# david-wb/tiny-diffusion

Hardware: AMD Instinct MI355X
Metric: train images/s (q_sample+fwd+MSE+bwd+allreduce+Adam), MNIST 28x28 UNet fp32; 1000-step sample latency in `sample` (higher is better)
Workload: dtype f32; 1 GPU; diffusion.py unconditional MNIST 28x28 UNet, fp32, train step, batch 256/GPU (BASELINE.json configs[1]); global_batch=256, per_gpu_batch=256, parallelism=dp1

## Files before the change

### tiny_diffusion_amd/csrc/unet.hip

```cpp
#include "internal.h"
#include <algorithm>
#include <cstdlib>
#include <mutex>
#include <new>
#include <string>
#include <vector>

namespace {

struct UnitDef {
  int cin, cout, hw;
  int in_bn;
  int cin_real;
};

struct NetSpec {
  int in_ch, hw0, out_hw;
  int x0_ch, x0_real;
  int overlap;
  int time_dim;
  int enc_hw[4];
  int dec_hw[3];
  int skip_ch[3];
  UnitDef units[13];
// ... 72 lines not shown
    bnscr = std::max(bnscr, tdx_bn_relu_bwd_scratch_floats((int64_t)b * d.hw * d.hw, d.cout));
    gbuf = std::max(gbuf, b * d.hw * d.hw * (size_t)std::max(d.cin, d.cout));
  }
  for (int k = 0; k < 3; ++k) {
    const int hp = S.enc_hw[k + 1];
    L.ep[k] = take(b * hp * hp * S.skip_ch[k]);
  }
  for (int k = 0; k < 3; ++k) {
    const UnitDef& d = S.units[7 + 2 * k];
    L.cat[k] = take(b * d.hw * d.hw * d.cin);
  }
  L.d1a = take(b * S.out_hw * S.out_hw * 64);
  gbuf = std::max(gbuf, b * (size_t)S.out_hw * S.out_hw * 64);
  L.stats = take(stats);
  L.ksplit_floats = ksplit;
  L.ksplit = take(ksplit);
  L.gbuf = gbuf;
  L.G1 = take(gbuf); L.G2 = take(gbuf); L.G3 = take(gbuf); L.G4 = take(gbuf);
  for (int k = 0; k < 3; ++k) {
    L.GS[k] = take(b * S.enc_hw[k] * S.enc_hw[k] * S.skip_ch[k]);
    L.gtp[k] = take(b * S.skip_ch[k]);
  }
  L.slabs = take(slabs);
  L.slabs2 = take(slabs);
  L.bnscr = take(bnscr);
  L.smallp = take((size_t)tdx_small_conv_wgrad_blocks(B, S.hw0, S.hw0) * tdx_small_conv_partial_width());
  L.smallp2 = take((size_t)tdx_small_conv_wgrad_blocks(B, S.hw0, S.hw0) * tdx_small_conv_partial_width());
  L.timescr = take(3 * b * S.time_dim);
  L.total = o;
  return L;
}

}

struct PlanHandles {
  hipStream_t side, side2, half;
  hipEvent_t ev[81];
};

struct tdx_unet {
  int max_batch, num_classes, kind;
  NetSpec spec_own;
  const NetSpec* spec;
  float* wpack;
  size_t wf_off[13], wd_off[13];
  float* upack;
  size_t uf_off[13], ud_off[13];
  bool wino_f[13], wino_d[13], wino_w[13];
  float* infer_ss;
  size_t iss_off[13];
  bool packed;
  bool wf_tiled;
  float* tab;
  size_t tab_floats;
  int tab_T, tab_batch, tab_gen, pack_gen;
  const void* tab_cond;
  const int64_t* tab_tau;
  bool skip_time_path;
  PStep ps;
  bool whole_batch;
  hipStream_t half_own;
  hipEvent_t ev_h_fork, ev_h_join;
  PlanHandles handles;
  int precision, saved_precision;
  int io16, saved_io16;
  tdx_allreduce_fn bn_sync;
  void* bn_sync_user;
  double* bn_sync_buf;
  int saved_batch, saved_mode;
  float* g_next;
  int bw_unit, bw_nblk;
  float* g_x;
  struct GBuf { float* p; int w_unit; int s2; int age; } gb[4];
  int clock;
  bool red_pending[13];
  bool materialize;
  int use_streams;
  hipStream_t side_own, side2_own;
  hipStream_t side;
  hipEvent_t ev_dy[13], ev_w[13], ev_join, ev_fork, ev_pack;
  hipStream_t side2;
  hipEvent_t ev_s2_fork[3], ev_s2_done[3], ev_join2, ev_red[13];
  hipEvent_t ev_mark[N_STAGES][2];
};

static std::mutex g_handles_mu;
static std::vector<PlanHandles> g_handles_pool;

static bool make_handles(PlanHandles* h) {
  {
    std::lock_guard<std::mutex> lk(g_handles_mu);
    if (!g_handles_pool.empty()) { *h = g_handles_pool.back(); g_handles_pool.pop_back(); return true; }
  }
  int lo = 0, hi = 0;
  (void)hipDeviceGetStreamPriorityRange(&lo, &hi);
  h->side = h->side2 = h->half = nullptr;
  if (hipStreamCreateWithPriority(&h->side, hipStreamNonBlocking, lo) != hipSuccess) return false;
  if (hipStreamCreateWithPriority(&h->side2, hipStreamNonBlocking, lo) != hipSuccess) return false;
  if (hipStreamCreateWithFlags(&h->half, hipStreamNonBlocking) != hipSuccess) return false;
  for (auto& e : h->ev)
    if (hipEventCreateWithFlags(&e, hipEventDisableTiming) != hipSuccess) return false;
  return true;
}

static void recycle_handles(const PlanHandles& h) {
  (void)hipStreamSynchronize(h.side);
  (void)hipStreamSynchronize(h.side2);
  (void)hipStreamSynchronize(h.half);
  std::lock_guard<std::mutex> lk(g_handles_mu);
  g_handles_pool.push_back(h);
}

extern "C" int tdx_unet_create_ex(tdx_unet** out, int max_batch, int kind, int num_classes) {
  return tdx_unet_create_hw(out, max_batch, kind, num_classes, 0);
}

extern "C" int tdx_unet_create_hw(tdx_unet** out, int max_batch, int kind, int num_classes, int hw) {
  return tdx_unet_create_full(out, max_batch, kind, num_classes, hw, 0);
}

extern "C" int tdx_unet_create_full(tdx_unet** out, int max_batch, int kind, int num_classes, int hw,
                                    int time_dim) {
  if (!out || max_batch <= 0 || num_classes < 0 || kind < 0 || kind > 2 || hw < 0 || time_dim < 0) return TDX_E_BADARG;
  if (kind == TDX_UNET_LATENT_MLP && time_dim != 0 && time_dim != 256) return TDX_E_SHAPE;
  if (kind == TDX_UNET_LAION && num_classes != 0) return TDX_E_BADARG;
  if (kind == TDX_UNET_LATENT_MLP && num_classes <= 0) return TDX_E_BADARG;
  NetSpec spec_hw;
  if (kind != TDX_UNET_LATENT_MLP) {
    if (!make_spec(kind, hw, time_dim, &spec_hw)) return TDX_E_SHAPE;
    const NetSpec& S = spec_hw;
    for (int i = 0; i < 13; ++i)
      if (!tdx_conv3x3_shape_ok(max_batch, S.units[i].hw, S.units[i].hw, S.units[i].cin, S.units[i].cout))
        return TDX_E_SHAPE;
  }
  tdx_unet* u = new (std::nothrow) tdx_unet();
  if (!u) return TDX_E_BADARG;
  u->max_batch = max_batch;
  u->num_classes = num_classes;
  u->kind = kind;
  if (kind != TDX_UNET_LATENT_MLP) u->spec_own = spec_hw;
  u->spec = kind == TDX_UNET_LATENT_MLP ? nullptr : &u->spec_own;
  size_t o = 64, so = 0;
  if (u->spec) {
    for (int i = 0; i < 13; ++i) {
      const UnitDef& d = u->spec->units[i];
      const size_t n = (size_t)d.cin * d.cout * 9;
      u->wf_off[i] = o; o += align64(n);
      u->wd_off[i] = o; o += align64(n);
      u->iss_off[i] = so; so += align64(2 * (size_t)d.cout);
    }
  } else {
    so = tdx_latent_infer_ss_floats();
  }
  hipError_t e = hipMalloc(&u->wpack, o * sizeof(float));
  if (e != hipSuccess) { delete u; return (int)e; }
  u->upack = nullptr;
  for (int i = 0; i < 13; ++i) u->wino_f[i] = u->wino_d[i] = u->wino_w[i] = false;
  if (u->spec) {
    size_t uo = 64;
    for (int i = 0; i < 13; ++i) {
      const size_t n = (size_t)u->spec->units[i].cin * u->spec->units[i].cout * 16;
      u->uf_off[i] = uo; uo += align64(n);
      u->ud_off[i] = uo; uo += align64(n);
    }
    e = hipMalloc(&u->upack, uo * sizeof(float));
    if (e != hipSuccess) { (void)hipFree(u->wpack); delete u; return (int)e; }
  }
  e = hipMalloc(&u->infer_ss, so * sizeof(float));
  if (e != hipSuccess) { (void)hipFree(u->wpack); if (u->upack) (void)hipFree(u->upack); delete u; return (int)e; }
  u->packed = false;
  u->wf_tiled = false;
  u->tab = nullptr;
  u->tab_floats = 0;
  u->tab_T = u->tab_batch = 0;
  u->tab_gen = -1;
  u->pack_gen = 0;
  u->tab_cond = nullptr;
  u->tab_tau = nullptr;
  u->skip_time_path = false;
  u->whole_batch = false;
  u->ps = {};
  u->precision = TDX_PREC_F32;
  u->saved_precision = TDX_PREC_F32;
  u->io16 = u->saved_io16 = 0;
  u->bn_sync = nullptr;
  u->bn_sync_user = nullptr;
  u->bn_sync_buf = nullptr;
  u->saved_batch = 0;
  u->saved_mode = -1;
  u->g_next = nullptr;
  u->g_x = nullptr;
  u->bw_unit = -1;
  u->bw_nblk = 0;
  u->materialize = g_knobs.materialize != 0;
  u->use_streams = g_knobs.streams < 0 ? (u->spec ? u->spec->overlap : 0) : g_knobs.streams;
  if (!make_handles(&u->handles)) {
    (void)hipFree(u->wpack); if (u->upack) (void)hipFree(u->upack); (void)hipFree(u->infer_ss);
    delete u;
    return TDX_E_STATE;
  }
  {
    const PlanHandles& h = u->handles;
    int k = 0;
    u->side_own = h.side; u->side2_own = h.side2; u->half_own = h.half;
    for (int i = 0; i < 13; ++i) { u->ev_dy[i] = h.ev[k++]; u->ev_w[i] = h.ev[k++]; u->ev_red[i] = h.ev[k++]; }
    for (int i = 0; i < 3; ++i) { u->ev_s2_fork[i] = h.ev[k++]; u->ev_s2_done[i] = h.ev[k++]; }
    u->ev_join = h.ev[k++]; u->ev_fork = h.ev[k++]; u->ev_pack = h.ev[k++]; u->ev_join2 = h.ev[k++];
    u->ev_h_fork = h.ev[k++]; u->ev_h_join = h.ev[k++];
    for (int i = 0; i < N_STAGES; ++i) { u->ev_mark[i][0] = h.ev[k++]; u->ev_mark[i][1] = h.ev[k++]; }
  }
  u->side = u->side_own;
  u->side2 = u->side2_own;
  *out = u;
  return 0;
}

extern "C" int tdx_unet_create(tdx_unet** out, int max_batch, int num_classes) {
  return tdx_unet_create_ex(out, max_batch, 0, num_classes);
}

extern "C" int tdx_unet_set_bn_sync(tdx_unet* u, tdx_allreduce_fn fn, void* user, double* buffer) {
  if (!u || (fn && !buffer)) return TDX_E_BADARG;
  if (!u->spec) return fn ? TDX_E_SHAPE : 0;
  u->bn_sync = fn;
  u->bn_sync_user = user;
  u->bn_sync_buf = buffer;
  return 0;
}

extern "C" int tdx_unet_set_streams(tdx_unet* u, int mode) {
  if (!u || mode < -1 || mode > 2) return TDX_E_BADARG;
  u->use_streams = mode < 0 ? (u->spec ? u->spec->overlap : 0) : mode;
  return 0;
}

extern "C" int tdx_unet_set_precision(tdx_unet* u, int precision) {
  if (!u || (precision != TDX_PREC_F32 && precision != TDX_PREC_BF16)) return TDX_E_BADARG;
  if (!u->spec) { u->precision = precision; return 0; }
  if (precision != u->precision) u->packed = false;
  u->precision = precision;
  u->io16 = precision == TDX_PREC_BF16 && g_knobs.bf16_storage ? 1 : 0;
  return 0;
}

extern "C" int tdx_unet_destroy(tdx_unet* u) {
  if (!u) return TDX_E_BADARG;
  recycle_handles(u->handles);
  (void)hipFree(u->wpack);
  if (u->upack) (void)hipFree(u->upack);
  (void)hipFree(u->infer_ss);
  if (u->tab) (void)hipFree(u->tab);
  delete u;
  return 0;
}

extern "C" size_t tdx_unet_workspace_bytes(const tdx_unet* u, int batch, int mode) {
  (void)mode;
  if (!u || batch <= 0 || batch > u->max_batch) return 0;
  if (!u->spec) return tdx_latent_workspace_floats(batch) * sizeof(float);
  const size_t whole = make_layout(*u->spec, batch).total;
  const int b0 = (batch + 1) / 2;
  const size_t halves = batch >= 2 ? make_layout(*u->spec, b0).total + make_layout(*u->spec, batch - b0).total : 0;
  return std::max(whole, halves) * sizeof(float);
}

extern "C" int tdx_unet_backward_stages(void) { return N_STAGES; }

extern "C" int tdx_unet_tensor(const tdx_unet* u, int batch, const char* name, size_t* offset_floats,
                               size_t* numel) {
  if (!u || !name || !offset_floats || !numel || batch <= 0 || batch > u->max_batch) return TDX_E_BADARG;
  if (!u->spec) return tdx_latent_tensor(batch, name, offset_floats, numel);
  const NetSpec& S = *u->spec;
  const Layout L = make_layout(S, batch);
  const size_t b = (size_t)batch;
  std::string n(name);
  auto unit_index = [&](const std::string& s, size_t prefix) -> int {
    if (s.size() <= prefix) return -1;
    int v = atoi(s.c_str() + prefix);
    return (v >= 0 && v < 13) ? v : -1;
  };
  auto sq = [](int v) { return (size_t)v * v; };
  struct { const char* nm; size_t off, cnt; } fixed[] = {
      {"x0", L.x0, b * sq(S.hw0) * S.x0_ch},
      {"e1p", L.ep[0], b * sq(S.enc_hw[1]) * S.skip_ch[0]},
      {"e2p", L.ep[1], b * sq(S.enc_hw[2]) * S.skip_ch[1]},
      {"e3p", L.ep[2], b * sq(S.enc_hw[3]) * S.skip_ch[2]},
      {"cat3", L.cat[0], b * sq(S.units[7].hw) * S.units[7].cin},
      {"cat2", L.cat[1], b * sq(S.units[9].hw) * S.units[9].cin},
      {"cat1", L.cat[2], b * sq(S.units[11].hw) * S.units[11].cin},
      {"d1a", L.d1a, b * sq(S.out_hw) * 64}, {"emb", L.emb, b * S.time_dim},
      {"t_copy", L.t, 2 * b}, {"tf", L.sin, b}, {"pre", L.pre, b * S.time_dim},
      {"time_g_h", L.timescr + 2 * b * S.time_dim, b * S.time_dim},
      {"t1", L.tp[0], b * S.skip_ch[0]}, {"t2", L.tp[1], b * S.skip_ch[1]}, {"t3", L.tp[2], b * S.skip_ch[2]},
      {"G1", L.G1, L.gbuf}, {"G2", L.G2, L.gbuf}, {"G3", L.G3, L.gbuf}, {"G4", L.G4, L.gbuf},
      {"GS1", L.GS[0], b * sq(S.enc_hw[0]) * S.skip_ch[0]},
// ... 43 lines not shown
    u->wino_d[i] = tdx_conv3x3_train_algo(B, d.hw, d.hw, d.cin, d.cout, 1) != 0;
    u->wino_w[i] = tdx_conv3x3_train_algo(B, d.hw, d.hw, d.cin, d.cout, 2) != 0;
  }
}

static int pack_units(tdx_unet* u, const float* const* P, int lo, int hi, tdx_stream_t stream, bool tiled, bool infer) {
  TdxPackBatch pb{};
  TdxWinoPackBatch wb{};
  for (int i = lo; i < hi; ++i) {
    const UnitDef& d = u->spec->units[i];
    const bool need_f = infer || !u->wino_f[i], need_d = !infer && !u->wino_d[i];
    if (need_f || need_d) {
      const int k = pb.count++;
      pb.w[k] = P[TDX_P_UNIT0 + 4 * i];
      pb.wf[k] = need_f ? u->wpack + u->wf_off[i] : nullptr;
      pb.wd[k] = need_d && !tiled ? u->wpack + u->wd_off[i] : nullptr;
      pb.cout[k] = d.cout; pb.cin[k] = d.cin; pb.cin_real[k] = d.cin_real;
    }
    if (u->wino_f[i] || u->wino_d[i]) {
      const int k = wb.count++;
      wb.w[k] = P[TDX_P_UNIT0 + 4 * i];
      wb.uf[k] = u->wino_f[i] ? u->upack + u->uf_off[i] : nullptr;
      wb.ud[k] = u->wino_d[i] ? u->upack + u->ud_off[i] : nullptr;
      wb.cout[k] = d.cout; wb.cin[k] = d.cin; wb.cin_real[k] = d.cin_real;
    }
  }
  if (pb.count) {
    auto pack = u->precision == TDX_PREC_BF16 ? tdx_pack_conv3x3_batch_bf16 : tiled ? tdx_pack_conv3x3_tiled_batch : tdx_pack_conv3x3_batch;
    int rc = pack(&pb, stream);
    if (rc) return rc;
  }
  if (wb.count) return tdx_pack_conv3x3_wino_batch(&wb, stream);
  return 0;
}

static int pack_impl(tdx_unet* u, const void* const* params, void* const* buffers,
                     tdx_stream_t stream, bool overlap = false, int train_batch = 0) {
  const float* const* P = reinterpret_cast<const float* const*>(params);
  if (!u->spec) {
    if (buffers) {
      int rc = tdx_latent_pack(P, buffers, u->infer_ss, to_stream(stream));
      if (rc) return rc;
    }
    u->packed = buffers != nullptr;
    ++u->pack_gen;
    return 0;
  }
  const bool tiled = buffers && !overlap && u->precision != TDX_PREC_BF16 && g_knobs.infer_ring;
  u->wf_tiled = tiled;
  decide_wino(u, train_batch, train_batch > 0);
  {
    int rc = pack_units(u, P, 0, overlap ? 2 : 13, stream, tiled, buffers != nullptr && !overlap);
    if (rc) return rc;
  }
  for (int i = 0; i < 13; ++i) {
    const UnitDef& d = u->spec->units[i];
    int rc = 0;
    if (buffers) {
      float* ss = u->infer_ss + u->iss_off[i];
      rc = tdx_bn_finalize(nullptr, 0, 0, 0, d.cout, P[TDX_P_UNIT0 + 4 * i + 2],
                           P[TDX_P_UNIT0 + 4 * i + 3], (float*)buffers[3 * i],
                           (float*)buffers[3 * i + 1], nullptr, ss, ss + d.cout, nullptr,
                           nullptr, 0, stream);
      if (rc) return rc;
    }
  }
  u->packed = buffers != nullptr;
  ++u->pack_gen;
  return 0;
}

extern "C" int tdx_unet_pack(tdx_unet* u, const void* const* params, void* const* buffers,
                             tdx_stream_t stream) {
  if (!u || !params || !buffers) return TDX_E_BADARG;
  return pack_impl(u, params, buffers, stream);
}

static int pack_tail(tdx_unet* u, const void* const* params, tdx_stream_t stream) {
  const float* const* P = reinterpret_cast<const float* const*>(params);
  TDX_HIP(hipEventRecord(u->ev_fork, to_stream(stream)));
  TDX_HIP(hipStreamWaitEvent(u->side, u->ev_fork, 0));
  int rc = pack_units(u, P, 2, 13, reinterpret_cast<tdx_stream_t>(u->side), false, false);
  if (rc) return rc;
  TDX_HIP(hipEventRecord(u->ev_pack, u->side));
  return 0;
}

#define RC(call)            \
  do {                      \
    int rc__ = (call);      \
    if (rc__) return rc__;  \
  } while (0)

static bool infer_halves(const tdx_unet* u, int batch, size_t workspace_bytes, int* b0) {
  if (!u->spec || !u->half_own || u->whole_batch || !g_knobs.sample_halves || batch < 2 || batch < g_knobs.sample_halves_min) return false;
  const int h0 = (batch + 1) / 2;
  if (workspace_bytes < (make_layout(*u->spec, h0).total + make_layout(*u->spec, batch - h0).total) * sizeof(float)) return false;
  *b0 = h0;
  return true;
}

static int unet_forward_impl(tdx_unet* u, const void* const* params, void* const* buffers, const float* x,
                             const int64_t* t, const void* cond, float* out, void* workspace, size_t workspace_bytes,
                             int batch, int mode, tdx_stream_t stream, const PStep& ps);

extern "C" int tdx_unet_forward(tdx_unet* u, const void* const* params, void* const* buffers,
                                const float* x, const int64_t* t, const void* cond, float* out,
                                void* workspace, size_t workspace_bytes, int batch, int mode,
                                tdx_stream_t stream) {
  if (!u || !params || !buffers || !x || !t || !out || !workspace) return TDX_E_BADARG;
  if (batch <= 0 || batch > u->max_batch) return TDX_E_BADARG;
  if (mode < TDX_MODE_TRAIN || mode > TDX_MODE_INFER) return TDX_E_BADARG;
  const bool needs_cond = u->kind == 1 || u->num_classes > 0;
  if (needs_cond != (cond != nullptr)) return TDX_E_BADARG;
  int b0 = 0;
  if (mode == TDX_MODE_INFER && infer_halves(u, batch, workspace_bytes, &b0)) {
    const NetSpec& S = *u->spec;
    if (!u->packed) RC(pack_impl(u, params, buffers, stream));
    hipStream_t st = to_stream(stream);
    const size_t per = (size_t)S.in_ch * S.hw0 * S.hw0;
    const size_t w0 = make_layout(S, b0).total;
    const void* cond1 = !cond ? nullptr
                        : u->kind == 1 ? static_cast<const void*>(static_cast<const float*>(cond) + (size_t)b0 * S.time_dim)
                                       : static_cast<const void*>(static_cast<const int64_t*>(cond) + b0);
    PStep ps0 = u->ps, ps1 = u->ps;
    if (ps1.x) {
      ps1.x += b0 * per;
      if (ps1.z) ps1.z += b0 * per;
      ps1.elem0 = (int64_t)(b0 * per);
      ps1.counter_dec = nullptr;
    }
    TDX_HIP(hipEventRecord(u->ev_h_fork, st));
    TDX_HIP(hipStreamWaitEvent(u->half_own, u->ev_h_fork, 0));
    RC(unet_forward_impl(u, params, buffers, x, t, cond, out, workspace, w0 * sizeof(float), b0, mode, stream, ps0));
    RC(unet_forward_impl(u, params, buffers, x + b0 * per, t + b0, cond1, out + b0 * per,
                         reinterpret_cast<float*>(workspace) + w0, workspace_bytes - w0 * sizeof(float), batch - b0, mode,
                         reinterpret_cast<tdx_stream_t>(u->half_own), ps1));
    TDX_HIP(hipEventRecord(u->ev_h_join, u->half_own));
    TDX_HIP(hipStreamWaitEvent(st, u->ev_h_join, 0));
    return 0;
  }
  return unet_forward_impl(u, params, buffers, x, t, cond, out, workspace, workspace_bytes, batch, mode, stream, u->ps);
}

static int unet_forward_impl(tdx_unet* u, const void* const* params, void* const* buffers, const float* x,
                             const int64_t* t, const void* cond, float* out, void* workspace, size_t workspace_bytes,
                             int batch, int mode, tdx_stream_t stream, const PStep& ps) {
  if (!u->spec) {
    if (workspace_bytes < tdx_latent_workspace_floats(batch) * sizeof(float)) return TDX_E_WORKSPACE;
    if (mode == TDX_MODE_INFER && !u->packed) {
      int rc = pack_impl(u, params, buffers, stream);
      if (rc) return rc;
    }
    int rc = tdx_latent_forward(reinterpret_cast<const float* const*>(params), buffers, x, t,
                                static_cast<const int64_t*>(cond), out, reinterpret_cast<float*>(workspace), batch,
                                mode, u->infer_ss, to_stream(stream), u->precision == TDX_PREC_BF16);
    if (rc) return rc;
    u->saved_batch = mode == TDX_MODE_INFER ? 0 : batch;
    u->saved_mode = mode;
    u->saved_precision = u->precision;
    return 0;
  }
  const NetSpec& S = *u->spec;
  const Layout L = make_layout(S, batch);
  if (workspace_bytes < L.total * sizeof(float)) return TDX_E_WORKSPACE;
  const float* const* P = reinterpret_cast<const float* const*>(params);
  float* ws = reinterpret_cast<float*>(workspace);
  hipStream_t st = to_stream(stream);
  u->side = u->use_streams == 1 ? u->side_own : st;
  u->side2 = u->use_streams ? u->side2_own : st;
  const int B = batch;
  const bool infer = mode == TDX_MODE_INFER;
  const bool training = mode == TDX_MODE_TRAIN;
  const int64_t* labels = u->kind == 0 ? static_cast<const int64_t*>(cond) : nullptr;
  const float* cond_emb = u->kind == 1 ? static_cast<const float*>(cond) : nullptr;

  const bool bf16 = u->precision == TDX_PREC_BF16;
  const int io16 = bf16 ? u->io16 : 0;
  if (!infer) RC(pack_impl(u, params, nullptr, stream, true, B));
  else if (!u->packed) RC(pack_impl(u, params, buffers, stream));
  if (!infer) {
    const size_t nx = (size_t)B * S.hw0 * S.hw0 * S.in_ch;
    const float* src[3] = {x, reinterpret_cast<const float*>(t), reinterpret_cast<const float*>(labels)};
    float* dst[3] = {ws + L.x, ws + L.t, ws + L.y};
    const size_t cnt[3] = {nx, 2 * (size_t)B, labels ? 2 * (size_t)B : 0};
    RC(tdx_copy_segments(src, dst, cnt, 3, st));
  }

  hipStream_t tst = st;
  if (!infer && u->side2 != st) {
    TDX_HIP(hipEventRecord(u->ev_fork, st));
    TDX_HIP(hipStreamWaitEvent(u->side2, u->ev_fork, 0));
    tst = u->side2;
  }
  if (!(infer && u->skip_time_path))
    RC(tdx_time_embed_fwd(u->kind, t, labels, cond_emb, P, ws + L.sin, ws + L.pre, ws + L.emb, ws + L.tp[0],
                          ws + L.tp[1], ws + L.tp[2], B, tst, S.time_dim));
  RC(tdx_initial_conv_fwd(x, P[TDX_P_INIT_W], P[TDX_P_INIT_B], ws + L.x0, B, S.hw0, S.hw0, S.in_ch,
                          S.x0_real, st, io16));

  auto sc = [&](int i) -> const float* { return infer ? nullptr : ws + L.ss[i]; };
  auto sh = [&](int i) -> const float* { return infer ? nullptr : ws + L.ss[i] + S.units[i].cout; };

  auto finalize_bn = [&](int i, int tiles, int tile_rows, int64_t count) -> int {
    const UnitDef& d = S.units[i];
    float* ss = ws + L.ss[i];
    if (training && u->bn_sync) {
      RC(tdx_bn_moments(ws + L.stats, tiles, tile_rows, count, d.cout, u->bn_sync_buf, st));
      RC(u->bn_sync(u->bn_sync_user, u->bn_sync_buf, 2 * d.cout + 1, stream));
      return tdx_bn_finalize_moments(u->bn_sync_buf, d.cout, P[TDX_P_UNIT0 + 4 * i + 2], P[TDX_P_UNIT0 + 4 * i + 3],
                                     (float*)buffers[3 * i], (float*)buffers[3 * i + 1], (int64_t*)buffers[3 * i + 2],
                                     ss, ss + d.cout, ss + 2 * d.cout, ss + 3 * d.cout, st);
    }
    return tdx_bn_finalize(ws + L.stats, tiles, tile_rows, count, d.cout, P[TDX_P_UNIT0 + 4 * i + 2],
                           P[TDX_P_UNIT0 + 4 * i + 3], (float*)buffers[3 * i], (float*)buffers[3 * i + 1],
                           (int64_t*)buffers[3 * i + 2], ss, ss + d.cout, ss + 2 * d.cout, ss + 3 * d.cout,
                           training ? 1 : 0, stream);
  };

  auto run_unit = [&](int i, const float* in, TdxSplitDefer* defer = nullptr, TdxPoolFuse* pool = nullptr) -> int {
    const UnitDef& d = S.units[i];
    const float* wf = u->wpack + u->wf_off[i];
    const float* bias = P[TDX_P_UNIT0 + 4 * i + 1];
    float* Y = ws + L.Y[i];
    float* ss = ws + L.ss[i];
    if (bf16) {
      const int64_t M = (int64_t)B * d.hw * d.hw;
      const bool mat16 = io16 && u->materialize && g_knobs.bf16_materialize;
      if (infer) {
        const float* iss = u->infer_ss + u->iss_off[i];
        return tdx_conv3x3_fwd_bf16_io(in, wf, bias, Y, B, d.hw, d.hw, d.cin, d.cout, TDX_CONV_OUT_BNRELU, nullptr,
                                       nullptr, iss, iss + d.cout, nullptr, io16, stream);
      }
      const bool on_load = d.in_bn && !mat16;
      if (d.in_bn && mat16) in = ws + L.A[i - 1];
      const int fl = (on_load ? TDX_CONV_IN_BNRELU : 0) | (training ? TDX_CONV_OUT_STATS : 0);
      RC(tdx_conv3x3_fwd_bf16_io(in, wf, bias, Y, B, d.hw, d.hw, d.cin, d.cout, fl, on_load ? sc(i - 1) : nullptr,
                                 on_load ? sh(i - 1) : nullptr, nullptr, nullptr, ws + L.stats, io16, stream));
      const int rows = tdx_conv3x3_bf16_stat_tile_rows();
      RC(finalize_bn(i, cdiv(M, rows), rows, M));
      if (mat16 && i + 1 < 13 && S.units[i + 1].in_bn)
        RC(tdx_bn_relu_apply(Y, ws + L.A[i], M, d.cout, ss, ss + d.cout, st, 1));
      return 0;
    }
    if (infer) {
      const float* iss = u->infer_ss + u->iss_off[i];
      if (u->wino_f[i] && tdx_conv3x3_infer_algo(B, d.hw, d.hw, d.cin, d.cout))
        return tdx_conv3x3_fwd_wino_infer_ex(in, u->upack + u->uf_off[i], bias, Y, B, d.hw, d.hw, d.cin, d.cout, iss,
                                             iss + d.cout, ws + L.G1, 2 * L.gbuf, stream, defer, pool);
      if (u->wf_tiled)
        return tdx_conv3x3_fwd_infer_ex(in, wf, bias, Y, B, d.hw, d.hw, d.cin, d.cout, iss, iss + d.cout, ws + L.G1,
                                        2 * L.gbuf, stream, defer, pool);
      return tdx_conv3x3_fwd_splitk_fused(in, wf, bias, Y, B, d.hw, d.hw, d.cin, d.cout, TDX_CONV_OUT_BNRELU, iss,
                                          iss + d.cout, ws + L.G1, 2 * L.gbuf, stream, defer, pool);
    }
    const bool bn_on_load = d.in_bn && !u->materialize;
    if (d.in_bn && u->materialize) in = ws + L.A[i - 1];
    int flags = (bn_on_load ? TDX_CONV_IN_BNRELU : 0) | (training ? TDX_CONV_OUT_STATS : 0);
    if (u->wino_f[i] && !bn_on_load) {
      RC(tdx_conv3x3_fwd_wino(in, u->upack + u->uf_off[i], bias, Y, B, d.hw, d.hw, d.cin, d.cout,
                              training ? TDX_CONV_OUT_STATS : 0, nullptr, nullptr, ws + L.stats, stream));
      RC(finalize_bn(i, tdx_conv3x3_wino_stat_tiles(B, d.hw, d.hw), tdx_conv3x3_wino_stat_tile_rows(B, d.hw, d.hw),
                     (int64_t)B * d.hw * d.hw));
      if (u->materialize && i + 1 < 13 && S.units[i + 1].in_bn)
        RC(tdx_bn_relu_apply(Y, ws + L.A[i], (int64_t)B * d.hw * d.hw, d.cout, ss, ss + d.cout, st));
      return 0;
    }
    if (bn_on_load)
      RC(tdx_conv3x3_fwd(in, wf, bias, Y, B, d.hw, d.hw, d.cin, d.cout, flags, sc(i - 1), sh(i - 1), nullptr, nullptr,
                         ws + L.stats, stream));
    else
      RC(tdx_conv3x3_fwd_train(in, wf, bias, Y, B, d.hw, d.hw, d.cin, d.cout, flags, ws + L.stats, ws + L.ksplit,
                               L.ksplit_floats, stream));
    const int tiles = tdx_conv3x3_stat_tiles(B, d.hw, d.hw, d.cin, d.cout);
    RC(finalize_bn(i, tiles, tdx_conv3x3_stat_tile_rows(B, d.hw, d.hw, d.cin, d.cout), (int64_t)B * d.hw * d.hw));
    if (u->materialize && i + 1 < 13 && S.units[i + 1].in_bn)
      RC(tdx_bn_relu_apply(Y, ws + L.A[i], (int64_t)B * d.hw * d.hw, d.cout, ss, ss + d.cout, st));
    return 0;
  };

  RC(run_unit(0, ws + L.x0));
  if (!infer) RC(pack_tail(u, params, stream));
  for (int k = 0; k < 3; ++k) {
    const int ua = 2 * k, ub = 2 * k + 1;
    if (k == 1 && !infer) TDX_HIP(hipStreamWaitEvent(st, u->ev_pack, 0));
    if (k > 0) RC(run_unit(ua, ws + L.ep[k - 1]));
    TdxPoolFuse pf{infer && !bf16 && (g_knobs.sample_fuse & 2) ? ws + L.ep[k] : nullptr};
    RC(run_unit(ub, ws + L.Y[ua], nullptr, pf.pooled ? &pf : nullptr));
    if (!infer) {
      const int kd = 2 - k, ud = 7 + 2 * kd;
      const UnitDef& dd = S.units[ud];
      const int c_up = S.units[kd == 0 ? 6 : 6 + 2 * kd].cout;
      TDX_HIP(hipEventRecord(u->ev_s2_fork[k], st));
      TDX_HIP(hipStreamWaitEvent(u->side2, u->ev_s2_fork[k], 0));
      RC(tdx_bilinear_ac_fwd_t(ws + L.Y[ub], sc(ub), sh(ub), ws + L.tp[k], ws + L.cat[kd], B, S.enc_hw[k],
                               S.enc_hw[k], dd.hw, dd.hw, S.skip_ch[k], dd.cin, c_up, io16,
                               reinterpret_cast<tdx_stream_t>(u->side2)));
      TDX_HIP(hipEventRecord(u->ev_s2_done[k], u->side2));
    }
    if (!pf.pooled)
      RC(tdx_maxpool2_ceil_fwd_t(ws + L.Y[ub], sc(ub), sh(ub), ws + L.ep[k], B, S.enc_hw[k], S.enc_hw[k],
                                 S.skip_ch[k], io16, stream));
  }
  const bool defer_ok = infer && !bf16 && (g_knobs.sample_fuse & 1);
  TdxSplitDefer dfr{};
  RC(run_unit(6, ws + L.ep[2], defer_ok ? &dfr : nullptr));
  for (int k = 0; k < 3; ++k) {
    const int ua = 7 + 2 * k, ub = 8 + 2 * k;
    const int prev = k == 0 ? 6 : 6 + 2 * k;
    const int skip_u = 5 - 2 * k;
    const int skip_k = 2 - k;
    const UnitDef& da = S.units[ua];
    const UnitDef& dp = S.units[prev];
    const int hw = da.hw, c_up = dp.cout, c_skip = S.skip_ch[skip_k];
    if (infer) {
      RC(tdx_bilinear_pair_fwd_ex(ws + L.Y[prev], &dfr, dp.hw, dp.hw, c_up, ws + L.Y[skip_u], ws + L.tp[skip_k],
                                  S.enc_hw[skip_k], S.enc_hw[skip_k], c_skip, ws + L.cat[k], B, hw, hw, st, io16));
      dfr = TdxSplitDefer{};
    } else {
      RC(tdx_bilinear_ac_fwd_t(ws + L.Y[prev], sc(prev), sh(prev), nullptr, ws + L.cat[k], B, dp.hw, dp.hw, hw, hw,
                               c_up, da.cin, 0, io16, stream));
      TDX_HIP(hipStreamWaitEvent(st, u->ev_s2_done[skip_k], 0));
    }
    RC(run_unit(ua, ws + L.cat[k]));
    RC(run_unit(ub, ws + L.Y[ua], defer_ok ? &dfr : nullptr));
  }
  if (dfr.splits > 0)
    RC(tdx_bilinear_pair_fwd_ex(nullptr, &dfr, S.dec_hw[2], S.dec_hw[2], 64, nullptr, nullptr, 0, 0, 0, ws + L.d1a, B,
                                S.out_hw, S.out_hw, st));
  else
    RC(tdx_bilinear_ac_fwd_t(ws + L.Y[12], sc(12), sh(12), nullptr, ws + L.d1a, B, S.dec_hw[2], S.dec_hw[2],
                             S.out_hw, S.out_hw, 64, 64, 0, io16, stream));
  if (infer && ps.x)
    RC(tdx_final_conv_fwd_psample(ws + L.d1a, P[TDX_P_FINAL_W], P[TDX_P_FINAL_B], out, B, S.out_hw, S.out_hw, S.in_ch,
                                  ps, st, io16));
  else
    RC(tdx_final_conv_fwd(ws + L.d1a, P[TDX_P_FINAL_W], P[TDX_P_FINAL_B], out, B, S.out_hw, S.out_hw, S.in_ch, st, io16));

  u->saved_batch = infer ? 0 : B;
  if (!infer) u->g_x = nullptr;
  u->saved_mode = mode;
  u->saved_precision = u->precision;
  u->saved_io16 = io16;
  return 0;
}

static int unet_backward_impl(tdx_unet* u, const void* const* params, void* const* grads, const float* d_out,
                              void* workspace, size_t workspace_bytes, int batch, int stage_lo, int stage_hi,
                              tdx_stream_t stream);

extern "C" int tdx_unet_backward(tdx_unet* u, const void* const* params, void* const* grads,
                                 const float* d_out, void* workspace, size_t workspace_bytes,
                                 int batch, int stage_lo, int stage_hi, tdx_stream_t stream) {
  if (!u || !params || !grads || !d_out || !workspace) return TDX_E_BADARG;
  const int rc = unet_backward_impl(u, params, grads, d_out, workspace, workspace_bytes, batch, stage_lo, stage_hi, stream);
  if (rc) u->g_x = nullptr;
  return rc;
}

static int unet_backward_impl(tdx_unet* u, const void* const* params, void* const* grads, const float* d_out,
                              void* workspace, size_t workspace_bytes, int batch, int stage_lo, int stage_hi,
                              tdx_stream_t stream) {
  if (batch != u->saved_batch || u->saved_mode == TDX_MODE_INFER || u->saved_mode < 0) return TDX_E_STATE;
  if (stage_lo < 0 || stage_hi > N_STAGES || stage_lo >= stage_hi) return TDX_E_BADARG;
  if (!u->spec) {
    if (workspace_bytes < tdx_latent_workspace_floats(batch) * sizeof(float)) return TDX_E_WORKSPACE;
    return tdx_latent_backward(reinterpret_cast<const float* const*>(params), reinterpret_cast<float* const*>(grads),
                               d_out, reinterpret_cast<float*>(workspace), batch,
                               u->saved_mode == TDX_MODE_TRAIN ? 1 : 0, stage_lo, stage_hi, u->num_classes,
                               to_stream(stream), u->saved_precision == TDX_PREC_BF16);
  }
  const NetSpec& S = *u->spec;
  const Layout L = make_layout(S, batch);
  if (workspace_bytes < L.total * sizeof(float)) return TDX_E_WORKSPACE;
  const float* const* P = reinterpret_cast<const float* const*>(params);
  float* const* G = reinterpret_cast<float* const*>(grads);
  float* ws = reinterpret_cast<float*>(workspace);
  hipStream_t st = to_stream(stream);
  u->side = u->use_streams == 1 ? u->side_own : st;
  u->side2 = u->use_streams ? u->side2_own : st;
  const int B = batch;
  const int training = u->saved_mode == TDX_MODE_TRAIN ? 1 : 0;
  if (u->precision != u->saved_precision) return TDX_E_STATE;
  const bool bf16 = u->saved_precision == TDX_PREC_BF16;
  const int io16 = u->saved_io16;
  typedef tdx_unet::GBuf GBuf;
  GBuf* gb = u->gb;
  int& clock = u->clock;
  if (stage_lo == 0) {
    float* base[4] = {ws + L.G1, ws + L.G2, ws + L.G3, ws + L.G4};
    for (int i = 0; i < 4; ++i) gb[i] = GBuf{base[i], -1, -1, 0};
    clock = 0;
    for (int i = 0; i < 13; ++i) u->red_pending[i] = false;
    u->bw_unit = -1;
  } else if (gb[0].p != ws + L.G1) {
    return TDX_E_STATE;
  }
  auto find = [&](const float* p) -> GBuf* {
    for (int i = 0; i < 4; ++i)
      if (gb[i].p == p) return &gb[i];
    return nullptr;
  };
  auto touch = [&](const float* p) { if (GBuf* b = find(p)) b->age = ++clock; };
  auto acquire = [&](const float* a, const float* b, float** out) -> int {
    GBuf* best = nullptr;
    for (int i = 0; i < 4; ++i) {
      GBuf& c = gb[i];
      if (c.p != a && c.p != b && (!best || c.age < best->age)) best = &c;
    }
    if (best->w_unit >= 0) TDX_HIP(hipStreamWaitEvent(st, u->ev_w[best->w_unit], 0));
    if (best->s2 >= 0) TDX_HIP(hipStreamWaitEvent(st, u->ev_s2_done[best->s2], 0));
    best->w_unit = -1;
    best->s2 = -1;
    best->age = ++clock;
    *out = best->p;
    return 0;
  };
  if (stage_lo > 0 && !find(u->g_next)) return TDX_E_STATE;
  float* g_next = u->g_next;

  tdx_stream_t side = reinterpret_cast<tdx_stream_t>(u->side);
  hipStreamCaptureStatus cap_status = hipStreamCaptureStatusNone;
  (void)hipStreamIsCapturing(st, &cap_status);
  const bool capturing = cap_status == hipStreamCaptureStatusActive;
  auto unit_bwd = [&](int i, const float* in, float** g_in_out) -> int {
    const UnitDef& d = S.units[i];
    float* g = g_next;
    const float* ss = ws + L.ss[i];
    const int64_t rows = (int64_t)B * d.hw * d.hw;
    if (u->bw_unit == i && u->bw_nblk > 0) {
      RC(tdx_bn_relu_bwd_tail(g, ws + L.Y[i], rows, d.cout, ss, ss + d.cout, ss + 2 * d.cout, ss + 3 * d.cout,
                              P[TDX_P_UNIT0 + 4 * i + 2], G[TDX_P_UNIT0 + 4 * i + 2], G[TDX_P_UNIT0 + 4 * i + 3],
                              G[TDX_P_UNIT0 + 4 * i + 1], ws + L.bnscr, u->bw_nblk,
                              ws + L.bnscr + (size_t)u->bw_nblk * 2 * d.cout, training,
                              training ? u->bn_sync : nullptr, u->bn_sync_user, u->bn_sync_buf, stream, io16));
    } else {
      RC(tdx_bn_relu_bwd_sync(g, ws + L.Y[i], rows, d.cout, ss, ss + d.cout, ss + 2 * d.cout,
                              ss + 3 * d.cout, P[TDX_P_UNIT0 + 4 * i + 2], G[TDX_P_UNIT0 + 4 * i + 2],
                              G[TDX_P_UNIT0 + 4 * i + 3], G[TDX_P_UNIT0 + 4 * i + 1], ws + L.bnscr, training,
                              training ? u->bn_sync : nullptr, u->bn_sync_user, u->bn_sync_buf, stream, io16));
    }
    u->bw_unit = -1;
    const bool mat = u->materialize && (!bf16 || (io16 && g_knobs.bf16_materialize));
    const bool bn_on_load = d.in_bn && !mat;
    if (d.in_bn && mat) in = ws + L.A[i - 1];
    const float* isc = bn_on_load ? ws + L.ss[i - 1] : nullptr;
    const float* ish = bn_on_load ? ws + L.ss[i - 1] + S.units[i - 1].cout : nullptr;
    const bool fork = true;
    float* slab = ws + ((i & 1) ? L.slabs2 : L.slabs);
    hipStream_t wst = fork ? u->side : st;
    hipStream_t red_st = capturing ? wst : u->side2;
    if (fork) {
      TDX_HIP(hipEventRecord(u->ev_dy[i], st));
      TDX_HIP(hipStreamWaitEvent(u->side, u->ev_dy[i], 0));
    }
    if (i + 2 < 13 && u->red_pending[i + 2]) {
      TDX_HIP(hipStreamWaitEvent(wst, u->ev_red[i + 2], 0));
      u->red_pending[i + 2] = false;
    }
    if (bf16)
      RC(tdx_conv3x3_wgrad_bf16_io(in, g, slab, B, d.hw, d.hw, d.cin, d.cout, bn_on_load ? TDX_CONV_IN_BNRELU : 0, isc,
                                   ish, io16, reinterpret_cast<tdx_stream_t>(wst)));
    else if (u->wino_w[i] && !bn_on_load)
      RC(tdx_conv3x3_wgrad_wino(in, g, slab, B, d.hw, d.hw, d.cin, d.cout, reinterpret_cast<tdx_stream_t>(wst)));
    else
      RC(tdx_conv3x3_wgrad(in, g, slab, B, d.hw, d.hw, d.cin, d.cout, bn_on_load ? TDX_CONV_IN_BNRELU : 0, isc, ish,
                           reinterpret_cast<tdx_stream_t>(wst)));
    TDX_HIP(hipEventRecord(u->ev_w[i], wst));
    if (red_st != wst) TDX_HIP(hipStreamWaitEvent(red_st, u->ev_w[i], 0));
    RC(tdx_conv3x3_wgrad_reduce_pad(slab, G[TDX_P_UNIT0 + 4 * i],
                                    bf16 ? tdx_conv3x3_wgrad_splits_bf16(B, d.hw, d.hw, d.cin, d.cout)
                                    : u->wino_w[i] && !bn_on_load ? tdx_conv3x3_wgrad_wino_splits(B, d.hw, d.hw, d.cin, d.cout)
                                                                  : tdx_conv3x3_wgrad_splits(B, d.hw, d.hw, d.cin, d.cout),
                                    d.cout, d.cin, d.cin_real, reinterpret_cast<tdx_stream_t>(red_st)));
    if (red_st != wst) {
      TDX_HIP(hipEventRecord(u->ev_red[i], red_st));
      u->red_pending[i] = true;
    }
    GBuf* gbuf = find(g);
    gbuf->w_unit = i;
    gbuf->age = ++clock;
    float* g_in;
    RC(acquire(g, nullptr, &g_in));
    if (bf16)
      RC(tdx_conv3x3_fwd_bf16_io(g, u->wpack + u->wd_off[i], nullptr, g_in, B, d.hw, d.hw, d.cout, d.cin, 0, nullptr,
                                 nullptr, nullptr, nullptr, nullptr, io16, stream));
    else if (u->wino_d[i])
      RC(tdx_conv3x3_fwd_wino(g, u->upack + u->ud_off[i], nullptr, g_in, B, d.hw, d.hw, d.cout, d.cin, 0, nullptr, nullptr,
                              nullptr, stream));
    else if (d.in_bn) {
      const float* pss = ws + L.ss[i - 1];
      int nblk = 0;
      RC(tdx_conv3x3_dgrad_bnbwd(g, u->wpack + u->wd_off[i], g_in, B, d.hw, d.hw, d.cout, d.cin, ws + L.Y[i - 1], pss,
                                 pss + d.cin, pss + 2 * d.cin, pss + 3 * d.cin, ws + L.bnscr, &nblk, ws + L.ksplit,
                                 L.ksplit_floats, stream));
      if (nblk > 0) { u->bw_unit = i - 1; u->bw_nblk = nblk; }
    } else
      RC(tdx_conv3x3_fwd_train(g, u->wpack + u->wd_off[i], nullptr, g_in, B, d.hw, d.hw, d.cout, d.cin, 0, nullptr,
                               ws + L.ksplit, L.ksplit_floats, stream));
    *g_in_out = g_in;
    return 0;
  };
  auto bw_y = [&](int i) -> const float* { return ws + L.Y[i]; };
  auto plain_unit_bwd = [&](int i, const float* in) -> int {
    float* g_in;
    RC(unit_bwd(i, in, &g_in));
    g_next = g_in;
    return 0;
  };
  auto ssc = [&](int i) { return ws + L.ss[i]; };
  auto ssh = [&](int i) { return ws + L.ss[i] + S.units[i].cout; };
  auto time_path_parts = [&](int parts) -> int {
    return tdx_time_embed_bwd(u->kind, u->num_classes > 0 ? reinterpret_cast<const int64_t*>(ws + L.y) : nullptr,
                              P, G, ws + L.sin, ws + L.pre, ws + L.emb, ws + L.gtp[0], ws + L.gtp[1],
                              ws + L.gtp[2], ws + L.timescr, B, u->num_classes, u->side2, S.time_dim, parts);
  };
  auto dec_level_bwd = [&](int k) -> int {
    const int ua = 7 + 2 * k;
    const int prev = k == 0 ? 6 : 6 + 2 * k;
    const int skip_k = 2 - k;
    const UnitDef& da = S.units[ua];
    const UnitDef& dp = S.units[prev];
    const int c_up = dp.cout, c_skip = S.skip_ch[skip_k];
    float* gcat;
    RC(unit_bwd(ua, ws + L.cat[k], &gcat));
    TDX_HIP(hipEventRecord(u->ev_s2_fork[k], st));
    TDX_HIP(hipStreamWaitEvent(u->side2, u->ev_s2_fork[k], 0));
    {
      int unused = 0;
      RC(tdx_bilinear_ac_bwd_bn(gcat, ws + L.GS[skip_k], B, S.enc_hw[skip_k], S.enc_hw[skip_k], da.hw, da.hw, c_skip,
                                da.cin, c_up, nullptr, nullptr, nullptr, nullptr, nullptr, nullptr, &unused,
                                reinterpret_cast<tdx_stream_t>(u->side2), io16));
    }
    RC(tdx_pixel_sum(ws + L.GS[skip_k], ws + L.gtp[skip_k], B, S.enc_hw[skip_k] * S.enc_hw[skip_k], c_skip,
                     u->side2, io16));
    TDX_HIP(hipEventRecord(u->ev_s2_done[k], u->side2));
    RC(tdx_time_proj_bwd(u->kind, skip_k, P, G, ws + L.emb, ws + L.gtp[skip_k], ws + L.timescr, B, u->side2,
                         S.time_dim));
    if (skip_k == 2) RC(time_path_parts(TDX_TIME_MID));
    find(gcat)->s2 = k;
    float* gup;
    RC(acquire(gcat, nullptr, &gup));
    {
      const float* pss = ws + L.ss[prev];
      int nblk = 0;
      RC(tdx_bilinear_ac_bwd_bn(gcat, gup, B, dp.hw, dp.hw, da.hw, da.hw, c_up, da.cin, 0, bw_y(prev), pss, pss + c_up,
                                pss + 2 * c_up, pss + 3 * c_up, ws + L.bnscr, &nblk, stream, io16));
      if (nblk > 0) { u->bw_unit = prev; u->bw_nblk = nblk; }
    }
    touch(gcat);
    g_next = gup;
    return 0;
  };
  auto time_path_bwd = [&](hipStream_t st) -> int {
    TDX_HIP(hipEventRecord(u->ev_fork, st));
    TDX_HIP(hipStreamWaitEvent(u->side2, u->ev_fork, 0));
    if (u->kind == 1) return 0;
    return time_path_parts(TDX_TIME_L1);
  };
  auto pooled_unit_bwd = [&](int ui, int k) -> int {
    float* gpool;
    RC(unit_bwd(ui, ws + L.ep[k], &gpool));
    const int ub = 2 * k + 1;
    float* gnew;
    RC(acquire(gpool, nullptr, &gnew));
    TDX_HIP(hipStreamWaitEvent(st, u->ev_s2_done[2 - k], 0));
    {
      const int cu = S.skip_ch[k];
      int nblk = 0;
      RC(tdx_maxpool2_ceil_bwd_bn(ws + L.Y[ub], ssc(ub), ssh(ub), gpool, ws + L.GS[k], gnew, B, S.enc_hw[k],
                                  S.enc_hw[k], cu, ws + L.ss[ub] + 2 * cu, ws + L.ss[ub] + 3 * cu,
                                  ws + L.bnscr, &nblk, stream, io16));
      if (nblk > 0) { u->bw_unit = ub; u->bw_nblk = nblk; }
    }
    touch(gpool);
    g_next = gnew;
    return 0;
  };

  for (int s = stage_lo; s < stage_hi; ++s) {
    switch (s) {
      case 0:
        TDX_HIP(hipEventRecord(u->ev_fork, st));
        TDX_HIP(hipStreamWaitEvent(u->side, u->ev_fork, 0));
        RC(tdx_final_conv_wgrad(ws + L.d1a, d_out, ws + L.smallp2, G[TDX_P_FINAL_W], G[TDX_P_FINAL_B], B,
                                S.out_hw, S.out_hw, S.in_ch, u->side, io16));
        {
          float *gd1a, *g12;
          RC(acquire(nullptr, nullptr, &gd1a));
          RC(tdx_final_conv_dgrad(d_out, P[TDX_P_FINAL_W], gd1a, B, S.out_hw, S.out_hw, S.in_ch, st, io16));
          if (S.dec_hw[2] == S.out_hw) {
            g_next = gd1a;
          } else {
            RC(acquire(gd1a, nullptr, &g12));
            const float* pss = ws + L.ss[12];
            int nblk = 0;
            RC(tdx_bilinear_ac_bwd_bn(gd1a, g12, B, S.dec_hw[2], S.dec_hw[2], S.out_hw, S.out_hw, 64, 64, 0, bw_y(12), pss,
                                      pss + 64, pss + 128, pss + 192, ws + L.bnscr, &nblk, stream, io16));
            if (nblk > 0) { u->bw_unit = 12; u->bw_nblk = nblk; }
            g_next = g12;
          }
        }
        break;
      case 1: RC(plain_unit_bwd(12, ws + L.Y[11])); break;
      case 2: RC(dec_level_bwd(2)); break;
      case 3: RC(plain_unit_bwd(10, ws + L.Y[9])); break;
      case 4: RC(dec_level_bwd(1)); break;
      case 5: RC(plain_unit_bwd(8, ws + L.Y[7])); break;
      case 6: RC(dec_level_bwd(0)); break;
      case 7: RC(pooled_unit_bwd(6, 2)); break;
      case 8: RC(plain_unit_bwd(5, ws + L.Y[4])); break;
      case 9: RC(pooled_unit_bwd(4, 1)); break;
      case 10: RC(plain_unit_bwd(3, ws + L.Y[2])); break;
      case 11: RC(pooled_unit_bwd(2, 0)); break;
      case 12: RC(plain_unit_bwd(1, ws + L.Y[0])); break;
      case 13: RC(plain_unit_bwd(0, ws + L.x0)); break;
      case 14:
        RC(time_path_bwd(st));
        RC(tdx_initial_conv_wgrad(ws + L.x, g_next, ws + L.smallp, G[TDX_P_INIT_W], G[TDX_P_INIT_B], B, S.hw0,
                                  S.hw0, S.in_ch, S.x0_real, st, io16));
        if (u->g_x) {
          RC(tdx_initial_conv_dgrad(g_next, P[TDX_P_INIT_W], u->g_x, B, S.hw0, S.hw0, S.in_ch, S.x0_real, st, io16));
          u->g_x = nullptr;
        }
        break;
    }
  }
  u->g_next = g_next;
  if (stage_hi == N_STAGES) return tdx_unet_backward_join(u, stream);
  return 0;
}

static int eval_step_impl(tdx_unet* u, const void* const* params, void* const* buffers, float* x, const void* cond,
                          PStep ps, int n_steps, int64_t* counter, int32_t* t_idx, int64_t* t_vec, float* eps,
                          int64_t n_elems, void* workspace, size_t workspace_bytes, int batch, tdx_stream_t stream,
                          int dyn_rank = 0, float dyn_frac = 0.f) {
  const int64_t* tau = ps.tau;
  const bool guided = ps.guided;
  if (!u || !params || !buffers || !x || !counter || !t_vec || !eps || !workspace || batch <= 0 || ps.t_idx != t_idx)
    return TDX_E_BADARG;
  if (const int rc = pstep_valid(ps, n_elems)) return rc;
  if (guided) {
    if (!u->spec) return TDX_E_SHAPE;
    if ((batch & 1) || 2 * n_elems != (int64_t)batch * u->spec->in_ch * u->spec->out_hw * u->spec->out_hw) return TDX_E_BADARG;
  }
  const bool tab = u->spec && u->tab && u->packed && u->tab_gen == u->pack_gen && u->tab_batch == batch &&
                   u->tab_cond == cond && u->tab_tau == tau && (!tau || u->tab_T == n_steps) && workspace &&
                   workspace_bytes >= make_layout(*u->spec, batch).total * sizeof(float);
  if (tab) {
// ... 196 lines not shown
```

Baseline: 27680 images/s.

## Elide redundant cross-stream waits, relax event fences, defer decoder wgrad reduce

Adds sequence counters for events recorded on the helper streams so the caller stream skips a wait when it has already waited on a later record from the same in-order helper stream. Most events are now created with the flag that disables the system-scope fence. For decoder concat units, the weight-gradient slab reduce is moved after the skip-gradient work on side2, so that side2 work is not queued behind the reduce (not applied while capturing). The aim is to cut stream-wait and event overhead and improve overlap. The risk is subtle correctness issues if the sequence bookkeeping misses a dependency.

```diff
diff --git a/tiny_diffusion_amd/csrc/unet.hip b/tiny_diffusion_amd/csrc/unet.hip
--- a/tiny_diffusion_amd/csrc/unet.hip
+++ b/tiny_diffusion_amd/csrc/unet.hip
@@ -178,7 +178,30 @@
   hipStream_t side2;
   hipEvent_t ev_s2_fork[3], ev_s2_done[3], ev_join2, ev_red[13];
   hipEvent_t ev_mark[N_STAGES][2];
+  struct Joined { hipStream_t st; bool capturing; uint64_t rec[2], seen[2]; } jn;
+  uint64_t seq_w[13], seq_s2[3], seq_pack;
 };
+
+static void caller_begin(tdx_unet* u, hipStream_t st, bool fresh) {
+  hipStreamCaptureStatus cs = hipStreamCaptureStatusNone;
+  (void)hipStreamIsCapturing(st, &cs);
+  const bool capturing = cs == hipStreamCaptureStatusActive;
+  if (fresh || st != u->jn.st || capturing != u->jn.capturing) u->jn.seen[0] = u->jn.seen[1] = 0;
+  u->jn.st = st;
+  u->jn.capturing = capturing;
+}
+
+static hipError_t helper_record(tdx_unet* u, int h, hipEvent_t ev, uint64_t* seq) {
+  *seq = ++u->jn.rec[h];
+  return hipEventRecord(ev, h ? u->side2 : u->side);
+}
+
+static hipError_t caller_wait(tdx_unet* u, hipStream_t st, int h, hipEvent_t ev, uint64_t seq) {
+  if ((h ? u->side2 : u->side) == st) return hipSuccess;
+  if (seq <= u->jn.seen[h]) return hipSuccess;
+  u->jn.seen[h] = seq;
+  return hipStreamWaitEvent(st, ev, 0);
+}
 
 static std::mutex g_handles_mu;
 static std::vector<PlanHandles> g_handles_pool;
@@ -194,8 +217,10 @@
   if (hipStreamCreateWithPriority(&h->side, hipStreamNonBlocking, lo) != hipSuccess) return false;
   if (hipStreamCreateWithPriority(&h->side2, hipStreamNonBlocking, lo) != hipSuccess) return false;
   if (hipStreamCreateWithFlags(&h->half, hipStreamNonBlocking) != hipSuccess) return false;
-  for (auto& e : h->ev)
-    if (hipEventCreateWithFlags(&e, hipEventDisableTiming) != hipSuccess) return false;
+  for (int i = 0; i < 81; ++i) {
+    const unsigned flags = hipEventDisableTiming | (i < 51 ? hipEventDisableSystemFence : 0);
+    if (hipEventCreateWithFlags(&h->ev[i], flags) != hipSuccess) return false;
+  }
   return true;
 }
 
@@ -307,6 +332,7 @@
   }
   u->side = u->side_own;
   u->side2 = u->side2_own;
+  u->jn = {};
   *out = u;
   return 0;
 }
@@ -516,7 +542,7 @@
   TDX_HIP(hipStreamWaitEvent(u->side, u->ev_fork, 0));
   int rc = pack_units(u, P, 2, 13, reinterpret_cast<tdx_stream_t>(u->side), false, false);
   if (rc) return rc;
-  TDX_HIP(hipEventRecord(u->ev_pack, u->side));
+  TDX_HIP(helper_record(u, 0, u->ev_pack, &u->seq_pack));
   return 0;
 }
 
@@ -622,6 +648,7 @@
   }
 
   hipStream_t tst = st;
+  if (!infer) caller_begin(u, st, true);
   if (!infer && u->side2 != st) {
     TDX_HIP(hipEventRecord(u->ev_fork, st));
     TDX_HIP(hipStreamWaitEvent(u->side2, u->ev_fork, 0));
@@ -717,7 +744,7 @@
   if (!infer) RC(pack_tail(u, params, stream));
   for (int k = 0; k < 3; ++k) {
     const int ua = 2 * k, ub = 2 * k + 1;
-    if (k == 1 && !infer) TDX_HIP(hipStreamWaitEvent(st, u->ev_pack, 0));
+    if (k == 1 && !infer) TDX_HIP(caller_wait(u, st, 0, u->ev_pack, u->seq_pack));
     if (k > 0) RC(run_unit(ua, ws + L.ep[k - 1]));
     TdxPoolFuse pf{infer && !bf16 && (g_knobs.sample_fuse & 2) ? ws + L.ep[k] : nullptr};
     RC(run_unit(ub, ws + L.Y[ua], nullptr, pf.pooled ? &pf : nullptr));
@@ -730,7 +757,7 @@
       RC(tdx_bilinear_ac_fwd_t(ws + L.Y[ub], sc(ub), sh(ub), ws + L.tp[k], ws + L.cat[kd], B, S.enc_hw[k],
                                S.enc_hw[k], dd.hw, dd.hw, S.skip_ch[k], dd.cin, c_up, io16,
                                reinterpret_cast<tdx_stream_t>(u->side2)));
-      TDX_HIP(hipEventRecord(u->ev_s2_done[k], u->side2));
+      TDX_HIP(helper_record(u, 1, u->ev_s2_done[k], &u->seq_s2[k]));
     }
     if (!pf.pooled)
       RC(tdx_maxpool2_ceil_fwd_t(ws + L.Y[ub], sc(ub), sh(ub), ws + L.ep[k], B, S.enc_hw[k], S.enc_hw[k],
@@ -754,7 +781,7 @@
     } else {
       RC(tdx_bilinear_ac_fwd_t(ws + L.Y[prev], sc(prev), sh(prev), nullptr, ws + L.cat[k], B, dp.hw, dp.hw, hw, hw,
                                c_up, da.cin, 0, io16, stream));
-      TDX_HIP(hipStreamWaitEvent(st, u->ev_s2_done[skip_k], 0));
+      TDX_HIP(caller_wait(u, st, 1, u->ev_s2_done[skip_k], u->seq_s2[skip_k]));
     }
     RC(run_unit(ua, ws + L.cat[k]));
     RC(run_unit(ub, ws + L.Y[ua], defer_ok ? &dfr : nullptr));
@@ -842,8 +869,8 @@
       GBuf& c = gb[i];
       if (c.p != a && c.p != b && (!best || c.age < best->age)) best = &c;
     }
-    if (best->w_unit >= 0) TDX_HIP(hipStreamWaitEvent(st, u->ev_w[best->w_unit], 0));
-    if (best->s2 >= 0) TDX_HIP(hipStreamWaitEvent(st, u->ev_s2_done[best->s2], 0));
+    if (best->w_unit >= 0) TDX_HIP(caller_wait(u, st, 0, u->ev_w[best->w_unit], u->seq_w[best->w_unit]));
+    if (best->s2 >= 0) TDX_HIP(caller_wait(u, st, 1, u->ev_s2_done[best->s2], u->seq_s2[best->s2]));
     best->w_unit = -1;
     best->s2 = -1;
     best->age = ++clock;
@@ -857,7 +884,27 @@
   hipStreamCaptureStatus cap_status = hipStreamCaptureStatusNone;
   (void)hipStreamIsCapturing(st, &cap_status);
   const bool capturing = cap_status == hipStreamCaptureStatusActive;
-  auto unit_bwd = [&](int i, const float* in, float** g_in_out) -> int {
+  caller_begin(u, st, false);
+  auto slab_reduce = [&](int i) -> int {
+    const UnitDef& d = S.units[i];
+    const bool mat = u->materialize && (!bf16 || (io16 && g_knobs.bf16_materialize));
+    const bool wino = u->wino_w[i] && !(d.in_bn && !mat);
+    float* slab = ws + ((i & 1) ? L.slabs2 : L.slabs);
+    hipStream_t wst = u->side;
+    hipStream_t red_st = capturing ? wst : u->side2;
+    if (red_st != wst) TDX_HIP(hipStreamWaitEvent(red_st, u->ev_w[i], 0));
+    RC(tdx_conv3x3_wgrad_reduce_pad(slab, G[TDX_P_UNIT0 + 4 * i],
+                                    bf16 ? tdx_conv3x3_wgrad_splits_bf16(B, d.hw, d.hw, d.cin, d.cout)
+                                    : wino ? tdx_conv3x3_wgrad_wino_splits(B, d.hw, d.hw, d.cin, d.cout)
+                                           : tdx_conv3x3_wgrad_splits(B, d.hw, d.hw, d.cin, d.cout),
+                                    d.cout, d.cin, d.cin_real, reinterpret_cast<tdx_stream_t>(red_st)));
+    if (red_st != wst) {
+      TDX_HIP(hipEventRecord(u->ev_red[i], red_st));
+      u->red_pending[i] = true;
+    }
+    return 0;
+  };
+  auto unit_bwd = [&](int i, const float* in, float** g_in_out, bool reduce_later = false) -> int {
     const UnitDef& d = S.units[i];
     float* g = g_next;
     const float* ss = ws + L.ss[i];
@@ -883,7 +930,6 @@
     const bool fork = true;
     float* slab = ws + ((i & 1) ? L.slabs2 : L.slabs);
     hipStream_t wst = fork ? u->side : st;
-    hipStream_t red_st = capturing ? wst : u->side2;
     if (fork) {
       TDX_HIP(hipEventRecord(u->ev_dy[i], st));
       TDX_HIP(hipStreamWaitEvent(u->side, u->ev_dy[i], 0));
@@ -900,17 +946,8 @@
     else
       RC(tdx_conv3x3_wgrad(in, g, slab, B, d.hw, d.hw, d.cin, d.cout, bn_on_load ? TDX_CONV_IN_BNRELU : 0, isc, ish,
                            reinterpret_cast<tdx_stream_t>(wst)));
-    TDX_HIP(hipEventRecord(u->ev_w[i], wst));
-    if (red_st != wst) TDX_HIP(hipStreamWaitEvent(red_st, u->ev_w[i], 0));
-    RC(tdx_conv3x3_wgrad_reduce_pad(slab, G[TDX_P_UNIT0 + 4 * i],
-                                    bf16 ? tdx_conv3x3_wgrad_splits_bf16(B, d.hw, d.hw, d.cin, d.cout)
-                                    : u->wino_w[i] && !bn_on_load ? tdx_conv3x3_wgrad_wino_splits(B, d.hw, d.hw, d.cin, d.cout)
-                                                                  : tdx_conv3x3_wgrad_splits(B, d.hw, d.hw, d.cin, d.cout),
-                                    d.cout, d.cin, d.cin_real, reinterpret_cast<tdx_stream_t>(red_st)));
-    if (red_st != wst) {
-      TDX_HIP(hipEventRecord(u->ev_red[i], red_st));
-      u->red_pending[i] = true;
-    }
+    TDX_HIP(helper_record(u, 0, u->ev_w[i], &u->seq_w[i]));
+    if (!reduce_later) RC(slab_reduce(i));
     GBuf* gbuf = find(g);
     gbuf->w_unit = i;
     gbuf->age = ++clock;
@@ -956,8 +993,9 @@
     const UnitDef& da = S.units[ua];
     const UnitDef& dp = S.units[prev];
     const int c_up = dp.cout, c_skip = S.skip_ch[skip_k];
+    const bool reduce_later = !capturing;
     float* gcat;
-    RC(unit_bwd(ua, ws + L.cat[k], &gcat));
+    RC(unit_bwd(ua, ws + L.cat[k], &gcat, reduce_later));
     TDX_HIP(hipEventRecord(u->ev_s2_fork[k], st));
     TDX_HIP(hipStreamWaitEvent(u->side2, u->ev_s2_fork[k], 0));
     {
@@ -968,7 +1006,8 @@
     }
     RC(tdx_pixel_sum(ws + L.GS[skip_k], ws + L.gtp[skip_k], B, S.enc_hw[skip_k] * S.enc_hw[skip_k], c_skip,
                      u->side2, io16));
-    TDX_HIP(hipEventRecord(u->ev_s2_done[k], u->side2));
+    TDX_HIP(helper_record(u, 1, u->ev_s2_done[k], &u->seq_s2[k]));
+    if (reduce_later) RC(slab_reduce(ua));
     RC(tdx_time_proj_bwd(u->kind, skip_k, P, G, ws + L.emb, ws + L.gtp[skip_k], ws + L.timescr, B, u->side2,
                          S.time_dim));
     if (skip_k == 2) RC(time_path_parts(TDX_TIME_MID));
@@ -998,7 +1037,7 @@
     const int ub = 2 * k + 1;
     float* gnew;
     RC(acquire(gpool, nullptr, &gnew));
-    TDX_HIP(hipStreamWaitEvent(st, u->ev_s2_done[2 - k], 0));
+    TDX_HIP(caller_wait(u, st, 1, u->ev_s2_done[2 - k], u->seq_s2[2 - k]));
     {
       const int cu = S.skip_ch[k];
       int nblk = 0;
```

Result: faster. 28070 images/s, median of 6 (+1.4%).
